# DeepRec-AI/HybridBackend

Hardware: AMD Instinct MI355X
Metric: M-lookups/sec, 26-col Criteo-shape dim16, 1/2/4/8 GPUs; % HBM roofline (higher is better)
Workload: dtype f32

## Files before the change

### hybridbackend_amd/_lib.py

```python
import ctypes as C
import os

_HERE = os.path.dirname(os.path.abspath(__file__))
LIB_PATH = os.environ.get('HBK_LIBRARY') or os.path.join(_HERE, 'lib', 'libhbk_core.so')

INT8, UINT8, INT32, UINT32, INT64, UINT64, HALF, FLOAT, DOUBLE = range(9)
APPLY_SGD, APPLY_ADAGRAD = 0, 2
APPLY_LAZY_ADAM, APPLY_FTRL, APPLY_ROWWISE_ADAGRAD = 3, 4, 5
GRAD_DETERMINISTIC = 1
COMBINER_SUM, COMBINER_MEAN, COMBINER_SQRTN = 0, 1, 2
OK, INVALID_ARGUMENT, UNIMPLEMENTED, INTERNAL = 0, 3, 12, 13
COMM_ID_BYTES = 128


class HbkError(RuntimeError):

  def __init__(self, code, message):
    super().__init__(f'[hbk status {code}] {message}')
    self.code = code


class InvalidArgumentError(HbkError, ValueError):
  pass

# ... 214 lines not shown


class StitchGradColumn(C.Structure):
  _fields_ = [('dim', C.c_int32), ('combiner', C.c_int32), ('n_ids', C.c_int64),
              ('index', C.c_void_p), ('row_splits', C.c_void_p), ('n_segments', C.c_int64),
              ('grad_out', C.c_void_p), ('grad_rows', C.c_void_p),
              ('run_start', C.c_void_p), ('run_base', C.c_void_p), ('n_runs', C.c_int32),
              ('grad_stride', C.c_int32), ('id_weights', C.c_void_p)]


_lib = None


def _declare(l):
  vp, i32, i64, sz = C.c_void_p, C.c_int32, C.c_int64, C.c_size_t
  protos = {
    'hbk_last_error': (C.c_char_p, []),
    'hbk_version': (C.c_char_p, []),
    'hbk_tables_layout': (C.c_size_t, [i32, vp, vp]),
    'hbk_tables_alloc': (C.c_int, [i32, vp, vp, vp]),
    'hbk_tables_free': (C.c_int, [vp]),
    'hbk_set_option': (C.c_int, [C.c_char_p, i32]),
    'hbk_get_option': (C.c_int, [C.c_char_p, vp]),
    'hbk_comm_rccl_ranks': (C.c_int, [vp]),
    'hbk_broadcast': (C.c_int, [vp, i32, vp, vp, i64, i32, vp]),
    'hbk_sharded_p2p_bind': (C.c_int, [vp, vp, vp, vp, vp]),
    'hbk_sharded_p2p_unbind': (C.c_int, [vp]),
    'hbk_sync_check': (C.c_int, []),
    'hbk_sync_check_stream': (C.c_int, [C.c_void_p]),
    'hbk_host_floormod_i64': (i64, [i64, i64]),
    'hbk_host_fastdiv_u64': (C.c_uint64, [C.c_uint64, C.c_uint64]),
    'hbk_host_crc32c': (C.c_uint32, [C.c_uint32, C.c_void_p, C.c_int64]),
    'hbk_host_xcd_contiguous': (i32, [i32, i32]),
    'hbk_floormod_n': (C.c_int, [i32, i32, vp, vp, vp, vp, vp]),
    'hbk_partition_workspace_bytes': (sz, [i32, vp, i32]),
    'hbk_partition_by_modulo_n': (C.c_int, [i32, i32, i32, vp, vp, vp, vp, vp, vp, sz, vp]),
    'hbk_partition_by_dual_modulo_n':
      (C.c_int, [i32, i32, i32, i32, i32, vp, vp, vp, vp, vp, vp, sz, vp]),
    'hbk_partition_by_modulo_host': (C.c_int, [i32, i32, i32, vp, vp, vp, vp, vp]),
    'hbk_partition_by_dual_modulo_host': (C.c_int, [i32, i32, i32, i32, i32, vp, vp, vp, vp, vp]),
    'hbk_cast_n': (C.c_int, [i32, i32, i32, vp, vp, vp, vp]),
    'hbk_unique_workspace_bytes': (sz, [i32, vp]),
    'hbk_unique_n': (C.c_int, [i32, vp, vp, vp, vp, vp, vp, sz, vp]),
    'hbk_group_lookup_fwd': (C.c_int, [i32, vp, vp]),
    'hbk_group_lookup_bwd_workspace_bytes': (sz, [i32, vp]),
    'hbk_group_lookup_bwd': (C.c_int, [i32, vp, C.c_float, vp, sz, vp]),
    'hbk_group_lookup_bwd_apply': (C.c_int, [i32, vp, i32, C.c_float, vp, sz, vp]),
    'hbk_group_lookup_bwd_adam_workspace_bytes': (sz, [i32, vp]),
    'hbk_group_lookup_bwd_adam': (C.c_int, [i32, vp, vp, vp, vp, C.c_float, vp, sz, vp]),
    'hbk_group_lookup_bwd_ftrl_workspace_bytes': (sz, [i32, vp]),
    'hbk_group_lookup_bwd_ftrl': (C.c_int, [i32, vp, vp, vp, vp, C.c_float, vp, sz, vp]),
    'hbk_group_lookup_fwd_clipped': (C.c_int, [i32, vp, vp, vp]),
    'hbk_group_lookup_bwd_apply_clipped_workspace_bytes': (sz, [i32, vp, vp]),
    'hbk_group_lookup_bwd_apply_clipped': (C.c_int, [i32, vp, vp, i32, C.c_float, vp, sz, vp]),
    'hbk_group_lookup_bwd_adam_clipped_workspace_bytes': (sz, [i32, vp, vp]),
    'hbk_group_lookup_bwd_adam_clipped': (C.c_int, [i32, vp, vp, vp, vp, vp, C.c_float, vp, sz, vp]),
    'hbk_group_lookup_bwd_ftrl_clipped_workspace_bytes': (sz, [i32, vp, vp]),
    'hbk_group_lookup_bwd_ftrl_clipped': (C.c_int, [i32, vp, vp, vp, vp, vp, C.c_float, vp, sz, vp]),
    'hbk_group_lookup_bwd_rowwise_adagrad_workspace_bytes': (sz, [i32, vp]),
    'hbk_group_lookup_bwd_rowwise_adagrad': (C.c_int, [i32, vp, vp, vp, C.c_float, vp, sz, vp]),
    'hbk_group_lookup_bwd_rowwise_adagrad_clipped_workspace_bytes': (sz, [i32, vp, vp]),
    'hbk_group_lookup_bwd_rowwise_adagrad_clipped': (C.c_int, [i32, vp, vp, vp, vp, C.c_float, vp, sz, vp]),
    'hbk_sparse_apply_slices_n': (C.c_int, [i32, vp, i32, vp, vp, vp, C.c_float, vp]),
    'hbk_lowp_lookup_fwd': (C.c_int, [i32, vp, vp]),
    'hbk_lowp_apply_slices_n': (C.c_int, [i32, vp, i32, vp, vp, vp, C.c_float, vp, vp]),
    'hbk_lowp_gather_rows_n': (C.c_int, [i32, vp, vp]),
# ... 254 lines not shown
```

### hybridbackend_amd/csrc/common.h

```cpp
#ifndef HBK_CSRC_COMMON_H_
#define HBK_CSRC_COMMON_H_

#include <hip/hip_runtime.h>
#include <stdarg.h>
#include <stdint.h>
#include <stdio.h>

#include "hbk.h"

namespace hbk {

int fail(int code, const char* fmt, ...);

#define HBK_HIP_OK(expr)                                                         \
  do {                                                                           \
    hipError_t e__ = (expr);                                                     \
    if (e__ != hipSuccess) {                                                     \
      return ::hbk::fail(HBK_INTERNAL, "%s failed: %s (%s:%d)", #expr,           \
                         hipGetErrorString(e__), __FILE__, __LINE__);            \
    }                                                                            \
  } while (0)

#define HBK_REQUIRE(cond, ...)                                                   \
  do {                                                                           \
// ... 51 lines not shown
  f.magic = m2 + 1;
  f.shift = k;
  f.kind = 2;
  return f;
}

__host__ __device__ inline uint64_t mulhi64(uint64_t a, uint64_t b) {
#if defined(__HIP_DEVICE_COMPILE__)
  return __umul64hi(a, b);
#else
  return (uint64_t)(((unsigned __int128)a * b) >> 64);
#endif
}

__host__ __device__ inline uint64_t fastdiv(uint64_t n, const FastDiv& f) {
  if (f.kind == 0) return n;
  if (f.kind == 1) return n >> f.shift;
  uint64_t t = mulhi64(f.magic, n);
  return (((n - t) >> 1) + t) >> f.shift;
}

__host__ __device__ inline uint64_t fastmod(uint64_t n, const FastDiv& f) {
  if (f.kind == 0) return 0;
  if (f.kind == 1) return n & (f.d - 1);
  return n - fastdiv(n, f) * f.d;
}

__host__ __device__ inline int xcd_contiguous(int b, int n, int on) {
  if (!on) return b;
  const int q = n >> 3, r = n & 7, x = b & 7, i = b >> 3;
  return (x < r ? x * (q + 1) : r * (q + 1) + (x - r) * q) + i;
}


__host__ __device__ inline uint64_t floormod_i64(int64_t v, const FastDiv& f) {
  uint64_t u = v < 0 ? (uint64_t)(~v) : (uint64_t)v;
  uint64_t r = fastmod(u, f);
  return v < 0 ? f.d - 1 - r : r;
}

struct Options {
  int bwd_buckets_log2 = -1;
  int bwd_bucket_pairs = 0;
  int bwd_split_pairs = 0;
  int bwd_onepass = 1;
  int fwd_xcd = 1;
  int bwd_xcd = 1;
  int bwd_wide = 1;
  int bwd_group_cols = 0;
  int bwd_dense = 1;
  int bwd_scatter_staged = 1;
  int bwd_rowsort_pos = 64;
  int bwd_pairs_packed = 1;
  int bwd_seg_inline = 1;
  int bwd_scale_fused = 1;
  int bwd_deterministic = 0;
  int bwd_simple = 1;
  int bwd_streams = 4;
  int bwd_lds_pad = 0;
  int bwd_trace = 0;
  int bwd_large_first = 0;
  int bwd_rowsort_ratio = 8;
  int bwd_weights_lds = 1;
  int fwd_d16 = 1;
  int fwd_interleave = 2;
  int fwd_hot_rows = 0;
  int unique_buckets_log2 = -1;
  int partition_sub_tiles = 1;
  int partition_fixed_max = 8;
  int partition_onepass = 1;
  int unique_onepass = 1;
  int sharded_groups = 0;
  int sharded_id64 = 0;
  int sharded_copy_self = 0;
  int sharded_trace = 0;
  int sharded_pack_early = 1;
  int sharded_wire_fused = 1;
  int sharded_inline = 1;
  int sharded_p2p = 1;
  int sharded_p2p_test_refuse = -1;
  int sync_wait_ms = 2000;
  int sync_onepass_off = 0;
  int sync_test_withhold = -1;
};
Options& options();

struct SyncTake {
  int32_t* words;
  int32_t* zero;
  int64_t zero_words;
  int32_t* status;
// ... 107 lines not shown
```

### hybridbackend_amd/csrc/lookup_bwd.hip

```cpp
#include <alloca.h>
#include <stdlib.h>
#include <string.h>

#include <algorithm>
#include <map>
#include <type_traits>
#include <mutex>
#include <vector>

#include "lookup_common.h"

namespace hbk {
size_t det_sort_temp_bytes(size_t n, int end_bit);
int det_sort_pairs(void* temp, size_t temp_bytes, const uint64_t* keys_in, uint64_t* keys_out,
                   const uint32_t* vals_in, uint32_t* vals_out, size_t n, int end_bit,
                   hipStream_t stream);
size_t det_scan_temp_bytes(size_t n);
int det_scan(void* temp, size_t temp_bytes, const int32_t* in, int32_t* out, size_t n,
             hipStream_t stream);
namespace {

constexpr int kBlock = 256;
constexpr int kWavesPerBlock = kBlock / kWave;
constexpr int kMaxCols = 64;
// ... 155 lines not shown
    rc.grad_delta = c.run_grads[rc.k] - start * c.dim;
  }
}

template <typename V>
__device__ inline void scale_segments(const GCol& c, const float* grad, int32_t stride, int combiner,
                                      int64_t s0, int n, const int32_t* sp) {
  constexpr int VE = sizeof(V) / 4;
  constexpr int kU = 4;
  const int tid = (int)threadIdx.x;
  const int sub = tid & ((1 << c.lpr_log2) - 1);
  const int groups = kBlock >> c.lpr_log2;
  if (sub >= c.chunks) return;
  for (int s = tid >> c.lpr_log2; s < n; s += kU * groups) {
    V g[kU];
    int32_t len[kU];
#pragma unroll
    for (int u = 0; u < kU; ++u) {
      const int ss = s + u * groups < n ? s + u * groups : n - 1;
      len[u] = s + u * groups < n ? sp[ss + 1] - sp[ss] : 0;
      g[u] = __builtin_nontemporal_load(reinterpret_cast<const V*>(
          grad + (s0 + ss) * (int64_t)stride + (int64_t)sub * VE));
    }
#pragma unroll
    for (int u = 0; u < kU; ++u) {
      if (len[u] <= 0) continue;
      const V v = combiner == HBK_COMBINER_MEAN ? g[u] / (float)len[u]
                                                : g[u] / sqrtf((float)len[u]);
      *reinterpret_cast<V*>(c.scaled + (s0 + s + u * groups) * (int64_t)c.dim + (int64_t)sub * VE) = v;
    }
  }
}

__device__ inline int32_t seg_search_wave(const int32_t* splits, int64_t n_seg, int32_t j) {
  const int lane = (int)threadIdx.x & (kWave - 1);
  int64_t lo = 0, n = n_seg;
  while (n > 1) {
    const int64_t step = (n + kWave - 1) / kWave;
    const int64_t s = lo + (int64_t)lane * step;
    const bool le = s < lo + n && splits[s] <= j;
    int k = (int)__builtin_popcountll(__ballot(le));
    if (k < 1) k = 1;
    const int64_t nlo = lo + (int64_t)(k - 1) * step;
    const int64_t rest = lo + n - nlo;
    lo = nlo;
    n = rest < step ? rest : step;
  }
  return (int32_t)lo;
}

__device__ inline int32_t tile_segments(const GCol& c, int64_t j_first, int64_t j_last,
                                        int32_t* seg_lds, int32_t* ends) {
  static_assert(kTile == kBlock * kPerThread && kPerThread % 4 == 0, "whole int4 per thread");
  const int tid = (int)threadIdx.x, lane = tid & (kWave - 1), wave = tid >> 6;
  if (wave == 0) {
    const int32_t s = seg_search_wave(c.splits, c.n_seg, (int32_t)j_first);
    if (tid == 0) ends[0] = s;
  } else if (wave == 1) {
    const int32_t s = seg_search_wave(c.splits, c.n_seg, (int32_t)j_last);
    if (tid == kWave) ends[1] = s;
  }
  int4* const v4 = reinterpret_cast<int4*>(seg_lds) + tid * (kPerThread / 4);
#pragma unroll
  for (int q = 0; q < kPerThread / 4; ++q) v4[q] = make_int4(0, 0, 0, 0);
  __syncthreads();
  const int32_t s_lo = ends[0], s_hi = ends[1];
  for (int32_t s = s_lo + 1 + tid; s <= s_hi; s += kBlock) {
    const int64_t p = (int64_t)c.splits[s] - j_first;
    if (p >= 0 && p < kTile) atomicAdd(&seg_lds[p], 1);
  }
  __syncthreads();
  int32_t x[kPerThread];
#pragma unroll
  for (int q = 0; q < kPerThread / 4; ++q) {
    const int4 v = v4[q];
    x[4 * q] = v.x;
    x[4 * q + 1] = v.y;
    x[4 * q + 2] = v.z;
    x[4 * q + 3] = v.w;
  }
#pragma unroll
  for (int q = 1; q < kPerThread; ++q) x[q] += x[q - 1];
  int32_t incl = x[kPerThread - 1];
#pragma unroll
  for (int o = 1; o < kWave; o <<= 1) {
    const int32_t y = __shfl_up(incl, o, kWave);
    if (lane >= o) incl += y;
  }
  if (lane == kWave - 1) ends[2 + wave] = incl;
  __syncthreads();
  int32_t before = incl - x[kPerThread - 1];
  for (int w = 0; w < wave; ++w) before += ends[2 + w];
#pragma unroll
  for (int q = 0; q < kPerThread / 4; ++q) {
    v4[q] = make_int4(x[4 * q] + before, x[4 * q + 1] + before, x[4 * q + 2] + before,
                      x[4 * q + 3] + before);
  }
  __syncthreads();
  return s_lo;
}

__global__ __launch_bounds__(kBlock) void bwd_segof_kernel(const GArgs a) {
  __shared__ int32_t sp[kBlock + 1];
  HBK_FIND_COL(a, segtile0)
  const int64_t s0 = ((int64_t)blockIdx.x - c.segtile0) * kBlock;
  const int tid = (int)threadIdx.x;
  const int n = c.n_seg - s0 < kBlock ? (int)(c.n_seg - s0) : kBlock;
  if (tid < n) sp[tid] = c.splits[s0 + tid];
  if (tid == 0) sp[n] = c.splits[s0 + n];
  __syncthreads();
  const int32_t lo = sp[0], hi = c.seg_of != nullptr ? sp[n] : sp[0];
  for (int32_t j = lo + tid; j < hi; j += kBlock) {
    int s = 0, e = n;
    while (e - s > 1) {
      const int mid = (s + e) >> 1;
      if (sp[mid] <= j) {
        s = mid;
      } else {
        e = mid;
      }
    }
    c.seg_of[j] = (int32_t)(s0 + s);
  }
  if (c.scaled != nullptr) {
    if (c.vec4) {
      scale_segments<f32x4>(c, c.grad_out, c.grad_stride, c.combiner, s0, n, sp);
    } else {
      scale_segments<float>(c, c.grad_out, c.grad_stride, c.combiner, s0, n, sp);
    }
  }
}
// ... 201 lines not shown
          seg[k] = c.seg_of[j];
        } else if (seg_inline) {
          seg[k] = s_lo + sp_lds[(k0 + k) * kBlock + tid];
        }
      }
    }
  };
  load_batch(0);
  for (int p = tid; p < P; p += kBlock) run[p] = c.bstart[p] + c.hist[(int64_t)ctile * P + p];
  __syncthreads();
  for (int k0 = 0; k0 < kPerThread; k0 += kBatch) {
    if (k0 > 0) load_batch(k0);
#pragma unroll
    for (int k = 0; k < kBatch; ++k) {
      const int64_t j = base + (int64_t)(k0 + k) * kBlock + tid;
      if (j < c.n_ids) {
        const uint64_t r = id_to_row(c.map, id[k]);
        if (r != kNoRow) {
          const int32_t pos = atomicAdd(&run[bucket_of(c, r)], 1);
          if (c.packed) {
            c.pair_row[0][pos] = (int64_t)((r << 32) | (uint64_t)(uint32_t)seg[k]);
          } else {
            c.pair_row[0][pos] = (int64_t)r;
            c.pair_seg[0][pos] = seg[k];
          }
        }
      }
    }
  }
}

constexpr int kStageMaxBuckets = 1024;

template <bool SIMPLE>
__global__ __launch_bounds__(kBlock, 4) void bwd_scatter_staged_kernel(const GArgs a) {
  extern __shared__ int32_t stage_dyn[];
  int32_t* const counters = stage_dyn;
  int32_t* const first = stage_dyn + a.stage_p;
  int32_t* const st_seg = stage_dyn + 2 * a.stage_p;
  __shared__ int64_t st_row[kTile];
  __shared__ uint16_t st_b[SIMPLE ? 1 : kTile];
  __shared__ int32_t wave_cnt[kWavesPerBlock];
  __shared__ int32_t n_staged;
  const int blk = xcd_contiguous((int)blockIdx.x, (int)gridDim.x, (a.xcd >> kXcdScatterBit) & 1);
  int ci;
  {
    const int l__ = (int)threadIdx.x & (kWave - 1);
    const int v__ = l__ < a.n_cols ? a.tile0[l__] : 0x7fffffff;
    ci = (int)__builtin_popcountll(__ballot(v__ <= blk)) - 1;
    ci = __builtin_amdgcn_readfirstlane(ci);
  }
  const GCol& c = a.col[ci];
  const int P = c.n_buckets;
  const int tid = (int)threadIdx.x, lane = tid & (kWave - 1), wave = tid >> 6;
  const int ctile = blk - c.tile0;
  const int64_t base = (int64_t)ctile * kTile;
  __shared__ int32_t seg_ends[2 + kWavesPerBlock];
  int32_t* const sp_lds = reinterpret_cast<int32_t*>(st_row);
  const bool seg_inline = c.splits != nullptr && (SIMPLE || c.seg_of == nullptr);
  RunCursor rc;
  int64_t id[kPerThread];
  int32_t seg[kPerThread];
#pragma unroll
  for (int k = 0; k < kPerThread; ++k) {
    const int64_t j = base + (int64_t)k * kBlock + tid;
    id[k] = 0;
    seg[k] = (int32_t)j;
    if (j < c.n_ids) {
      if (!SIMPLE && c.n_runs > 0) {
        run_seek(c, j, rc);
        if (!c.det) seg[k] = (int32_t)(uint32_t)(rc.grad_delta + j * c.dim);
      }
      id[k] = load_id(c.ids, SIMPLE ? 1 : c.ids64, SIMPLE ? j : j + rc.id_delta);
      if (!SIMPLE && c.seg_of != nullptr) seg[k] = c.seg_of[j];
    }
  }
  const int per = (P + kBlock - 1) / kBlock;
  const int beg = tid * per;
  const int end = beg + per < P ? beg + per : P;
  int32_t gpos[kStageMaxBuckets / kBlock];
#pragma unroll
  for (int q = 0; q < kStageMaxBuckets / kBlock; ++q) {
    const int p = beg + q;
    gpos[q] = q < per && p < end ? c.bstart[p] + c.hist[(int64_t)ctile * P + p] : 0;
  }
  if (seg_inline) {
    const int64_t j_last = (base + kTile < c.n_ids ? base + kTile : c.n_ids) - 1;
    const int32_t s_lo = tile_segments(c, base, j_last, sp_lds, seg_ends);
#pragma unroll
    for (int k = 0; k < kPerThread; ++k) seg[k] = s_lo + sp_lds[k * kBlock + tid];
  }
  for (int p = tid; p < P; p += kBlock) counters[p] = 0;
  __syncthreads();
  int32_t br[kPerThread];
#pragma unroll
  for (int k = 0; k < kPerThread; ++k) {
    const int64_t j = base + (int64_t)k * kBlock + tid;
    br[k] = -1;
    if (j < c.n_ids) {
      const uint64_t r = id_to_row(c.map, id[k]);
      id[k] = (int64_t)r;
      if (r != kNoRow) {
        const int b = SIMPLE ? (int)__umulhi((uint32_t)r, c.dense_mul) : bucket_of(c, r);
        br[k] = b | (atomicAdd(&counters[b], 1) << 10);
      }
    }
  }
  __syncthreads();
  int32_t sum_c = 0;
#pragma unroll
  for (int q = 0; q < kStageMaxBuckets / kBlock; ++q) {
    if (q < per && beg + q < end) sum_c += counters[beg + q];
  }
  int32_t incl_c = sum_c;
#pragma unroll
  for (int off = 1; off < kWave; off <<= 1) {
    const int32_t w = __shfl_up(incl_c, off, kWave);
    if (lane >= off) incl_c += w;
  }
  if (lane == kWave - 1) wave_cnt[wave] = incl_c;
  __syncthreads();
  int32_t run_c = incl_c - sum_c;
  for (int w = 0; w < wave; ++w) run_c += wave_cnt[w];
#pragma unroll
  for (int q = 0; q < kStageMaxBuckets / kBlock; ++q) {
    const int p = beg + q;
    if (q < per && p < end) {
      const int32_t n_c = counters[p];
      first[p] = run_c;
      counters[p] = gpos[q] - run_c;
      run_c += n_c;
    }
  }
  if (tid == kBlock - 1) n_staged = run_c;
  __syncthreads();
#pragma unroll
  for (int k = 0; k < kPerThread; ++k) {
    if (br[k] >= 0) {
      const int b = br[k] & 1023;
      const int L = first[b] + (br[k] >> 10);
      if (SIMPLE || c.packed) {
        st_row[L] = (int64_t)(((uint64_t)id[k] << 32) | (uint64_t)(uint32_t)seg[k]);
      } else {
        st_row[L] = id[k];
        st_seg[L] = seg[k];
      }
      if (!SIMPLE) st_b[L] = (uint16_t)b;
    }
  }
  __syncthreads();
  const int n_st = n_staged;
#pragma unroll
  for (int k = 0; k < kPerThread; ++k) {
    const int L = k * kBlock + tid;
    if (L < n_st) {
      const int sb = SIMPLE ? (int)__umulhi((uint32_t)((uint64_t)st_row[L] >> 32), c.dense_mul) : (int)st_b[L];
      const int32_t pos = counters[sb] + L;
      c.pair_row[0][pos] = st_row[L];
      if (!SIMPLE && !c.packed) c.pair_seg[0][pos] = st_seg[L];
    }
  }
}

#ifdef HBK_BWD_STAMPS
__device__ unsigned long long g_grp_trace[kTraceBlocks * kTraceSlots];
#define HBK_GSTAMP(i)                                                                       \
  do {                                                                                      \
    if (threadIdx.x == 0 && blockIdx.x < kTraceBlocks) {                                    \
      g_grp_trace[blockIdx.x * kTraceSlots + (i)] = __builtin_amdgcn_s_memrealtime();       \
    }                                                                                       \
  } while (0)
#else
#define HBK_GSTAMP(i)
#endif

constexpr int kGroupMaxBuckets = 2 * kBlock;

struct GSync {
  int32_t* hist;
  int32_t* zero;
  int64_t zero_words;
  SyncWait wait;
};

template <bool SIMPLE>
__global__ __launch_bounds__(kBlock, 4) void bwd_group_kernel(const GArgs a, const GSync y) {
  __shared__ int32_t counters[kGroupMaxBuckets];
  __shared__ int32_t tot_s[kGroupMaxBuckets], pre_s[kGroupMaxBuckets];
  __shared__ int64_t st_row[kTile];
  extern __shared__ int32_t st_seg[];
  __shared__ uint16_t st_b[kTile];
  __shared__ int32_t wave_tot[kWavesPerBlock], wave_cnt[kWavesPerBlock];
  __shared__ int32_t n_extra, gave_up, n_staged;
  const int tid = (int)threadIdx.x, lane = tid & (kWave - 1), wave = tid >> 6;
// ... 2358 lines not shown
    const unsigned tiles_p = (unsigned)((total + kDetTile - 1) / kDetTile);
    hipLaunchKernelGGL(det_heads_kernel, dim3(tiles_p), dim3(kBlock), 0, stream, a);
    HBK_HIP_OK(hipGetLastError());
    rc = det_scan(ws + l.temp, l.temp_bytes, heads, ranks, (size_t)total, stream);
    if (rc != HBK_OK) return rc;
    if (vec4) {
      det_launch_reduce<f32x4>(a, max_dim / 4, stream);
    } else {
      det_launch_reduce<float>(a, max_dim, stream);
    }
    HBK_HIP_OK(hipGetLastError());
    hipLaunchKernelGGL(det_counts_kernel, dim3(1), dim3(kWave), 0, stream, a);
    HBK_HIP_OK(hipGetLastError());
  }
  return HBK_OK;
}

}
}

#ifdef HBK_BWD_STAMPS
extern "C" int hbk_debug_grp_trace(unsigned long long* out, int reset) {
  using namespace hbk;
  HBK_HIP_OK(hipDeviceSynchronize());
  if (out != nullptr) {
    HBK_HIP_OK(hipMemcpyFromSymbol(out, HIP_SYMBOL(g_grp_trace), sizeof(g_grp_trace)));
  }
  if (reset) {
    static unsigned long long z[kTraceBlocks * kTraceSlots];
    HBK_HIP_OK(hipMemcpyToSymbol(HIP_SYMBOL(g_grp_trace), z, sizeof(z)));
  }
  return HBK_OK;
}
extern "C" int hbk_debug_bwd_sub(unsigned long long* out) {
  using namespace hbk;
  HBK_HIP_OK(hipDeviceSynchronize());
  HBK_HIP_OK(hipMemcpyFromSymbol(out, HIP_SYMBOL(g_bwd_sub), sizeof(g_bwd_sub)));
  return HBK_OK;
}
extern "C" int hbk_debug_bwd_trace(unsigned long long* out, int reset) {
  using namespace hbk;
  HBK_HIP_OK(hipDeviceSynchronize());
  if (out != nullptr) {
    HBK_HIP_OK(hipMemcpyFromSymbol(out, HIP_SYMBOL(g_bwd_trace), sizeof(g_bwd_trace)));
  }
  if (reset) {
    static unsigned long long z[kTraceBlocks * kTraceSlots];
    HBK_HIP_OK(hipMemcpyToSymbol(HIP_SYMBOL(g_bwd_trace), z, sizeof(z)));
  }
  return HBK_OK;
}
#endif

extern "C" size_t hbk_group_lookup_bwd_workspace_bytes(int32_t n_cols,
                                                       const hbk_lookup_grad_column_t* cols) {
  if (n_cols <= 0 || cols == nullptr) return 0;
  if (hbk::any_weighted(n_cols, cols)) {
    std::vector<hbk_lookup_grad_column_t> as_sum;
    const size_t tb = hbk::weighted_as_sum(n_cols, cols, nullptr, &as_sum);
    return tb + hbk_group_lookup_bwd_workspace_bytes(n_cols, as_sum.data());
  }
  std::vector<hbk::ColInfo> info;
  for (int32_t c = 0; c < n_cols; ++c) info.push_back(hbk::col_info(cols[c]));
  return hbk::call_layout(n_cols, cols, info).total;
}

// ... 383 lines not shown
                   c.dense_mul != 0;
    unpacked = unpacked || c.packed == 0;
  }
  const size_t lds_tail = (unpacked ? (size_t)kTile * 4 : 0) + (size_t)options().bwd_lds_pad * 1024;
  memset(sync, 0, sizeof(*sync));
  const auto group_kernel = simple_group ? &bwd_group_kernel<true> : &bwd_group_kernel<false>;
  bool onepass = g.onepass && g.sync_words < (1ll << 30);
  if (onepass) {
    SyncTake take;
    onepass = sync_take(ls, (size_t)g.sync_words, &take, reinterpret_cast<const void*>(group_kernel), kBlock,
                        64, caller);
    if (onepass) {
      sync->hist = take.words;
      sync->zero = take.zero;
      sync->zero_words = take.zero_words;
      sync->wait = sync_wait_of(take);
    }
  }
  if (onepass) {
    SyncChain chain(ls);
    hipLaunchKernelGGL(group_kernel, tiles, block, lds_tail, ls, args, *sync);
    return true;
  }
  hipLaunchKernelGGL(simple_group ? &bwd_hist_kernel<true> : &bwd_hist_kernel<false>, tiles, block, g.lds_hist,
                     ls, args);
  if (g.small_scan) {
    hipLaunchKernelGGL(bwd_scan_fused_kernel, dim3((unsigned)k), block, 0, ls, args);
  } else {
    hipLaunchKernelGGL(bwd_scan_tiles_kernel, dim3((unsigned)g.scans), block, 0, ls, args);
    hipLaunchKernelGGL(bwd_scan_kernel, dim3((unsigned)k), block, 0, ls, args);
  }
  if (g.lds_hist <= (size_t)4 * kStageMaxBuckets && options().bwd_scatter_staged != 0) {
    args.stage_p = (int32_t)(g.lds_hist / 4);
    hipLaunchKernelGGL(simple_group ? &bwd_scatter_staged_kernel<true> : &bwd_scatter_staged_kernel<false>,
                       tiles, block, 2 * g.lds_hist + lds_tail, ls, args);
  } else {
    hipLaunchKernelGGL(bwd_scatter_pairs_kernel, tiles, block, g.lds_hist, ls, args);
  }
  return false;
}

int launch_reduce_merge(const Group& g, bool det, int32_t apply, float apply_lr, const int4* desc,
                        const int32_t* poison, hipStream_t ls) {
  const GArgs& args = g.args;
  const int step = apply_lr == 0.0f ? 0 : apply == HBK_APPLY_ADAGRAD ? 2 : 1;
  typedef void (*reduce_fn)(const GArgs, const int4*, int, int, const int32_t*);
  typedef void (*merge_fn)(const GArgs, int, const int32_t*);
#define HBK_BY_STEP(K, V, ...) {&K<V, 0, ##__VA_ARGS__>, &K<V, 1, ##__VA_ARGS__>, &K<V, 2, ##__VA_ARGS__>}
  static const reduce_fn kReduce[kKinds][3] = {
      HBK_BY_STEP(bwd_dense_kernel, f32x4, false), HBK_BY_STEP(bwd_dense_kernel, float, false),
      HBK_BY_STEP(bwd_dense_kernel, f32x4, true), HBK_BY_STEP(bwd_dense_kernel, float, true),
      HBK_BY_STEP(bwd_reduce_kernel, f32x4, false), HBK_BY_STEP(bwd_reduce_kernel, float, false),
      {nullptr, &bwd_reduce_kernel<f32x4, 1, true>, &bwd_reduce_kernel<f32x4, 2, true>},
      {nullptr, &bwd_reduce_kernel<float, 1, true>, &bwd_reduce_kernel<float, 2, true>},
      HBK_BY_STEP(bwd_rowsort_kernel, f32x4), HBK_BY_STEP(bwd_rowsort_kernel, float)};
  static const merge_fn kMerge[kKinds][3] = {
      HBK_BY_STEP(bwd_dense_merge_kernel, f32x4), HBK_BY_STEP(bwd_dense_merge_kernel, float),
      HBK_BY_STEP(bwd_dense_merge_kernel, f32x4), HBK_BY_STEP(bwd_dense_merge_kernel, float),
      HBK_BY_STEP(bwd_merge_kernel, f32x4, false), HBK_BY_STEP(bwd_merge_kernel, float, false),
      {nullptr, &bwd_merge_kernel<f32x4, 1, true>, &bwd_merge_kernel<f32x4, 2, true>},
      {nullptr, &bwd_merge_kernel<float, 1, true>, &bwd_merge_kernel<float, 2, true>},
      HBK_BY_STEP(bwd_rowsort_merge_kernel, f32x4), HBK_BY_STEP(bwd_rowsort_merge_kernel, float)};
  static const reduce_fn kReduceDet[2][3] = {HBK_BY_STEP(bwd_rowsort_kernel, f32x4, true),
                                             HBK_BY_STEP(bwd_rowsort_kernel, float, true)};
#undef HBK_BY_STEP
  int status = HBK_OK;
  if (det) {
    hipLaunchKernelGGL(bwd_rowsort_count_kernel, dim3((unsigned)g.buckets), dim3(kBlock), 0, ls, args, desc,
// ... 229 lines not shown
```

### hybridbackend_amd/csrc/misc.cpp

```cpp
#include <stdlib.h>
#include <string.h>

#include <vector>

#include "common.h"

namespace hbk {
namespace {
thread_local char g_last_error[1024] = "";
}

int fail(int code, const char* fmt, ...) {
  va_list ap;
  va_start(ap, fmt);
  vsnprintf(g_last_error, sizeof(g_last_error), fmt, ap);
  va_end(ap);
  return code;
}
}

namespace hbk {
namespace {
struct OptionEntry {
  const char* name;
  const char* env;
  int Options::*field;
};
const OptionEntry kOptions[] = {
    {"bwd_buckets_log2", "HBK_BWD_LOG2P", &Options::bwd_buckets_log2},
    {"bwd_bucket_pairs", "HBK_BWD_TARGET", &Options::bwd_bucket_pairs},
    {"bwd_split_pairs", "HBK_BWD_SPLIT", &Options::bwd_split_pairs},
    {"bwd_onepass", "HBK_BWD_ONEPASS", &Options::bwd_onepass},
    {"bwd_group_cols", "HBK_BWD_GROUP_COLS", &Options::bwd_group_cols},
    {"bwd_dense", "HBK_BWD_DENSE", &Options::bwd_dense},
    {"bwd_scatter_staged", "HBK_BWD_SCATTER_STAGED", &Options::bwd_scatter_staged},
    {"bwd_rowsort_pos", "HBK_BWD_ROWSORT_POS", &Options::bwd_rowsort_pos},
    {"bwd_rowsort_ratio", "HBK_BWD_ROWSORT_RATIO", &Options::bwd_rowsort_ratio},
    {"bwd_deterministic", "HBK_BWD_DETERMINISTIC", &Options::bwd_deterministic},
    {"bwd_streams", "HBK_BWD_STREAMS", &Options::bwd_streams},
    {"bwd_trace", "HBK_BWD_TRACE", &Options::bwd_trace},
    {"bwd_lds_pad", "HBK_BWD_LDS_PAD", &Options::bwd_lds_pad},
    {"bwd_large_first", "HBK_BWD_LARGE_FIRST", &Options::bwd_large_first},
    {"bwd_pairs_packed", "HBK_BWD_PAIRS_PACKED", &Options::bwd_pairs_packed},
    {"bwd_seg_inline", "HBK_BWD_SEG_INLINE", &Options::bwd_seg_inline},
    {"bwd_scale_fused", "HBK_BWD_SCALE_FUSED", &Options::bwd_scale_fused},
    {"bwd_simple", "HBK_BWD_SIMPLE", &Options::bwd_simple},
    {"fwd_d16", "HBK_FWD_D16", &Options::fwd_d16},
    {"bwd_weights_lds", "HBK_BWD_WEIGHTS_LDS", &Options::bwd_weights_lds},
    {"bwd_wide", "HBK_BWD_WIDE", &Options::bwd_wide},
    {"bwd_xcd", "HBK_BWD_XCD", &Options::bwd_xcd},
    {"fwd_xcd", "HBK_FWD_XCD", &Options::fwd_xcd},
    {"fwd_hot_rows", "HBK_FWD_HOT", &Options::fwd_hot_rows},
    {"fwd_interleave", "HBK_FWD_INTERLEAVE", &Options::fwd_interleave},
    {"unique_buckets_log2", "HBK_UNIQUE_LOG2P", &Options::unique_buckets_log2},
    {"partition_sub_tiles", "HBK_PART_SUB", &Options::partition_sub_tiles},
    {"partition_fixed_max", "HBK_PART_FIXED", &Options::partition_fixed_max},
    {"partition_onepass", "HBK_PART_ONEPASS", &Options::partition_onepass},
    {"unique_onepass", "HBK_UNIQUE_ONEPASS", &Options::unique_onepass},
    {"sharded_groups", "HBK_SHARDED_GROUPS", &Options::sharded_groups},
    {"sharded_id64", "HBK_SHARDED_ID64", &Options::sharded_id64},
    {"sharded_copy_self", "HBK_SHARDED_COPY_SELF", &Options::sharded_copy_self},
    {"sharded_trace", "HBK_SHARDED_TRACE", &Options::sharded_trace},
    {"sharded_inline", "HBK_SHARDED_INLINE", &Options::sharded_inline},
    {"sharded_p2p", "HBK_SHARDED_P2P", &Options::sharded_p2p},
    {"sharded_p2p_test_refuse", "HBK_SHARDED_P2P_TEST_REFUSE", &Options::sharded_p2p_test_refuse},
    {"sharded_wire_fused", "HBK_SHARDED_WIRE_FUSED", &Options::sharded_wire_fused},
    {"sharded_pack_early", "HBK_SHARDED_PACK_EARLY", &Options::sharded_pack_early},
    {"sync_wait_ms", "HBK_SYNC_WAIT_MS", &Options::sync_wait_ms},
// ... 71 lines not shown
  if (n == 0) return HBK_OK;
  std::vector<size_t> off((size_t)n);
  const size_t total = hbk_tables_layout(n, bytes, off.data());
  void* p = nullptr;
  const hipError_t e = hipMalloc(&p, total > 0 ? total : 1);
  if (e != hipSuccess) {
    (void)hipGetLastError();
    return fail(HBK_INTERNAL, "tables_alloc: hipMalloc of %zu bytes failed: %s", total,
                hipGetErrorString(e));
  }
  for (int32_t i = 0; i < n; ++i) tables[i] = static_cast<char*>(p) + off[(size_t)i];
  *slab = p;
  return HBK_OK;
}
extern "C" int hbk_tables_free(void* slab) {
  using namespace hbk;
  if (slab == nullptr) return HBK_OK;
  const hipError_t e = hipFree(slab);
  if (e != hipSuccess) return fail(HBK_INTERNAL, "tables_free: %s", hipGetErrorString(e));
  return HBK_OK;
}

extern "C" int64_t hbk_host_floormod_i64(int64_t v, int64_t d) {
  if (d <= 0) return -1;
  hbk::FastDiv f = hbk::make_fastdiv((uint64_t)d);
  f.d = (uint64_t)d;
  return (int64_t)hbk::floormod_i64(v, f);
}

extern "C" int32_t hbk_host_xcd_contiguous(int32_t block, int32_t n_blocks) {
  return hbk::xcd_contiguous(block, n_blocks, 1);
}

extern "C" uint64_t hbk_host_fastdiv_u64(uint64_t n, uint64_t d) {
  if (d == 0) return 0;
  hbk::FastDiv f = hbk::make_fastdiv(d);
  return hbk::fastdiv(n, f);
}

extern "C" uint32_t hbk_host_crc32c(uint32_t crc, const void* data, int64_t n) {
  struct Tables {
    uint32_t t[8][256];
    Tables() {
      for (uint32_t i = 0; i < 256; ++i) {
        uint32_t c = i;
        for (int k = 0; k < 8; ++k) c = (c & 1u) ? (c >> 1) ^ 0x82f63b78u : c >> 1;
        t[0][i] = c;
      }
      for (uint32_t i = 0; i < 256; ++i) {
        for (int s = 1; s < 8; ++s) t[s][i] = (t[s - 1][i] >> 8) ^ t[0][t[s - 1][i] & 0xffu];
      }
    }
  };
  static const Tables tab;
  const uint8_t* p = static_cast<const uint8_t*>(data);
  uint32_t l = ~crc;
  if (p == nullptr || n <= 0) return crc;
  while (n > 0 && (reinterpret_cast<uintptr_t>(p) & 7u) != 0) {
    l = tab.t[0][(l ^ *p++) & 0xffu] ^ (l >> 8);
    --n;
  }
  while (n >= 8) {
    uint64_t w;
    memcpy(&w, p, 8);
    const uint32_t lo = (uint32_t)w ^ l, hi = (uint32_t)(w >> 32);
    l = tab.t[7][lo & 0xffu] ^ tab.t[6][(lo >> 8) & 0xffu] ^ tab.t[5][(lo >> 16) & 0xffu] ^
// ... 12 lines not shown
```

### include/hbk.h

```cpp
#ifndef HBK_H_
#define HBK_H_

#include <stddef.h>
#include <stdint.h>

#ifdef __cplusplus
extern "C" {
#endif

typedef void* hbk_stream_t;

#define HBK_OK 0
#define HBK_INVALID_ARGUMENT 3
#define HBK_UNIMPLEMENTED 12
#define HBK_INTERNAL 13

#define HBK_INT8 0
#define HBK_UINT8 1
#define HBK_INT32 2
#define HBK_UINT32 3
#define HBK_INT64 4
#define HBK_UINT64 5
#define HBK_HALF 6
#define HBK_FLOAT 7
#define HBK_DOUBLE 8

#define HBK_COMBINER_SUM 0
#define HBK_COMBINER_MEAN 1
#define HBK_COMBINER_SQRTN 2

#define HBK_TOPOLOGY_ALL 0
#define HBK_TOPOLOGY_INTRA_NODE 1
#define HBK_TOPOLOGY_INTER_NODE 2

const char* hbk_last_error(void);
const char* hbk_version(void);

size_t hbk_tables_layout(int32_t n, const size_t* bytes, size_t* offsets);
int hbk_tables_alloc(int32_t n, const size_t* bytes, void** tables, void** slab);
int hbk_tables_free(void* slab);
int hbk_set_option(const char* name, int32_t value);
int hbk_get_option(const char* name, int32_t* value);
int hbk_sync_check(void);
int hbk_sync_check_stream(hbk_stream_t stream);
int64_t hbk_host_floormod_i64(int64_t v, int64_t d);
uint64_t hbk_host_fastdiv_u64(uint64_t n, uint64_t d);
int32_t hbk_host_xcd_contiguous(int32_t block, int32_t n_blocks);
uint32_t hbk_host_crc32c(uint32_t crc, const void* data, int64_t n);

int hbk_floormod_n(int32_t n_cols, int32_t dtype, const void* const* inputs,
                   const int64_t* lens, const int64_t* buckets, void* const* outputs,
                   hbk_stream_t stream);

size_t hbk_partition_workspace_bytes(int32_t n_cols, const int64_t* lens,
                                     int32_t num_partitions);
int hbk_partition_by_modulo_n(int32_t n_cols, int32_t dtype, int32_t num_partitions,
                              const void* const* inputs, const int64_t* lens,
                              void* const* outputs, int32_t* const* sizes,
                              int32_t* const* indices, void* workspace,
                              size_t workspace_bytes, hbk_stream_t stream);

int hbk_partition_by_dual_modulo_n(int32_t n_cols, int32_t dtype, int32_t num_partitions,
                                   int32_t modulus, int32_t stage,
                                   const void* const* inputs, const int64_t* lens,
                                   void* const* outputs, int32_t* const* sizes,
                                   int32_t* const* indices, void* workspace,
                                   size_t workspace_bytes, hbk_stream_t stream);
int hbk_partition_by_modulo_host(int32_t n_cols, int32_t dtype, int32_t num_partitions,
                                 const void* const* inputs, const int64_t* lens,
                                 void* const* outputs, int32_t* const* sizes,
                                 int32_t* const* indices);
int hbk_partition_by_dual_modulo_host(int32_t n_cols, int32_t dtype, int32_t num_partitions,
                                      int32_t modulus, int32_t stage,
                                      const void* const* inputs, const int64_t* lens,
                                      void* const* outputs, int32_t* const* sizes,
                                      int32_t* const* indices);

int hbk_cast_n(int32_t n, int32_t src_dtype, int32_t dst_dtype, const void* const* inputs,
               const int64_t* lens, void* const* outputs, hbk_stream_t stream);

// ... 694 lines not shown
```

Measured before the change: 30630.

## Make staged backward scatter kernel persistent with next-tile prefetch

Converts the staged backward scatter kernel from one block per tile into a persistent grid sized to the resident block count. Each block walks several tiles using an XCD-aware walk, strided by default. In the simple path it issues the next tile's id loads and segment search while the current tile is being written out, to hide load latency. It also raises the launch-bounds occupancy hint and swaps the shuffle-based scan for ds_bpermute. This adds register pressure, loop and synchronisation overhead, and gives up some parallelism when there are few tiles.

```diff
diff --git a/hybridbackend_amd/_lib.py b/hybridbackend_amd/_lib.py
--- a/hybridbackend_amd/_lib.py
+++ b/hybridbackend_amd/_lib.py
@@ -270,6 +270,7 @@
     'hbk_host_fastdiv_u64': (C.c_uint64, [C.c_uint64, C.c_uint64]),
     'hbk_host_crc32c': (C.c_uint32, [C.c_uint32, C.c_void_p, C.c_int64]),
     'hbk_host_xcd_contiguous': (i32, [i32, i32]),
+    'hbk_host_persistent_walk': (None, [i32, i32, i32, i32, i32, vp]),
     'hbk_floormod_n': (C.c_int, [i32, i32, vp, vp, vp, vp, vp]),
     'hbk_partition_workspace_bytes': (sz, [i32, vp, i32]),
     'hbk_partition_by_modulo_n': (C.c_int, [i32, i32, i32, vp, vp, vp, vp, vp, vp, sz, vp]),
diff --git a/hybridbackend_amd/csrc/common.h b/hybridbackend_amd/csrc/common.h
--- a/hybridbackend_amd/csrc/common.h
+++ b/hybridbackend_amd/csrc/common.h
@@ -107,6 +107,32 @@
   return (x < r ? x * (q + 1) : r * (q + 1) + (x - r) * q) + i;
 }
 
+struct ItemWalk {
+  int first, step, count;
+};
+__host__ __device__ inline ItemWalk persistent_walk(int b, int grid, int n, int on, int contiguous) {
+  int xs = 0, len = n, w = grid, i = b;
+  if (on && grid >= 8) {
+    const int q = n >> 3, r = n & 7, x = b & 7;
+    i = b >> 3;
+    xs = x < r ? x * (q + 1) : r * (q + 1) + (x - r) * q;
+    len = q + (x < r ? 1 : 0);
+    w = (grid >> 3) + (x < (grid & 7) ? 1 : 0);
+  }
+  ItemWalk k;
+  if (contiguous) {
+    const int lo = (int)((long long)i * len / w), hi = (int)((long long)(i + 1) * len / w);
+    k.first = xs + lo;
+    k.step = 1;
+    k.count = hi - lo;
+  } else {
+    k.first = xs + i;
+    k.step = w;
+    k.count = i < len ? (len - i + w - 1) / w : 0;
+  }
+  return k;
+}
+
 
 __host__ __device__ inline uint64_t floormod_i64(int64_t v, const FastDiv& f) {
   uint64_t u = v < 0 ? (uint64_t)(~v) : (uint64_t)v;
@@ -132,6 +158,7 @@
   int bwd_deterministic = 0;
   int bwd_simple = 1;
   int bwd_streams = 4;
+  int bwd_scatter_walk = 0;
   int bwd_lds_pad = 0;
   int bwd_trace = 0;
   int bwd_large_first = 0;
diff --git a/hybridbackend_amd/csrc/lookup_bwd.hip b/hybridbackend_amd/csrc/lookup_bwd.hip
--- a/hybridbackend_amd/csrc/lookup_bwd.hip
+++ b/hybridbackend_amd/csrc/lookup_bwd.hip
@@ -211,8 +211,8 @@
   }
 }
 
-__device__ inline int32_t seg_search_wave(const int32_t* splits, int64_t n_seg, int32_t j) {
-  const int lane = (int)threadIdx.x & (kWave - 1);
+__device__ inline int32_t seg_search_wave(const int32_t* splits, int64_t n_seg, int32_t j,
+                                          int lane = (int)threadIdx.x & (kWave - 1)) {
   int64_t lo = 0, n = n_seg;
   while (n > 1) {
     const int64_t step = (n + kWave - 1) / kWave;
@@ -228,22 +228,38 @@
   return (int32_t)lo;
 }
 
-__device__ inline int32_t tile_segments(const GCol& c, int64_t j_first, int64_t j_last,
-                                        int32_t* seg_lds, int32_t* ends) {
-  static_assert(kTile == kBlock * kPerThread && kPerThread % 4 == 0, "whole int4 per thread");
-  const int tid = (int)threadIdx.x, lane = tid & (kWave - 1), wave = tid >> 6;
+__device__ inline void tile_segment_ends(const GCol& c, int64_t j_first, int64_t j_last, int32_t* ends,
+                                         int tid = (int)threadIdx.x) {
+  const int wave = tid >> 6, lane = tid & (kWave - 1);
   if (wave == 0) {
-    const int32_t s = seg_search_wave(c.splits, c.n_seg, (int32_t)j_first);
+    const int32_t s = seg_search_wave(c.splits, c.n_seg, (int32_t)j_first, lane);
     if (tid == 0) ends[0] = s;
   } else if (wave == 1) {
-    const int32_t s = seg_search_wave(c.splits, c.n_seg, (int32_t)j_last);
+    const int32_t s = seg_search_wave(c.splits, c.n_seg, (int32_t)j_last, lane);
     if (tid == kWave) ends[1] = s;
   }
+}
+
+__device__ inline void tile_segments_clear(int32_t* seg_lds, int tid = (int)threadIdx.x) {
+  static_assert(kTile == kBlock * kPerThread && kPerThread % 4 == 0, "whole int4 per thread");
   int4* const v4 = reinterpret_cast<int4*>(seg_lds) + tid * (kPerThread / 4);
 #pragma unroll
   for (int q = 0; q < kPerThread / 4; ++q) v4[q] = make_int4(0, 0, 0, 0);
-  __syncthreads();
-  const int32_t s_lo = ends[0], s_hi = ends[1];
+}
+
+__device__ inline int32_t wave_inclusive_sum(int32_t v, int lane) {
+#pragma unroll
+  for (int o = 1; o < kWave; o <<= 1) {
+    const int32_t y = __builtin_amdgcn_ds_bpermute((lane >= o ? lane - o : lane) << 2, v);
+    if (lane >= o) v += y;
+  }
+  return v;
+}
+
+__device__ inline void tile_segment_counts(const GCol& c, int64_t j_first, int32_t s_lo, int32_t s_hi,
+                                           int32_t* seg_lds, int32_t* wave_tot, int tid = (int)threadIdx.x) {
+  const int lane = tid & (kWave - 1), wave = tid >> 6;
+  int4* const v4 = reinterpret_cast<int4*>(seg_lds) + tid * (kPerThread / 4);
   for (int32_t s = s_lo + 1 + tid; s <= s_hi; s += kBlock) {
     const int64_t p = (int64_t)c.splits[s] - j_first;
     if (p >= 0 && p < kTile) atomicAdd(&seg_lds[p], 1);
@@ -260,22 +276,26 @@
   }
 #pragma unroll
   for (int q = 1; q < kPerThread; ++q) x[q] += x[q - 1];
-  int32_t incl = x[kPerThread - 1];
-#pragma unroll
-  for (int o = 1; o < kWave; o <<= 1) {
-    const int32_t y = __shfl_up(incl, o, kWave);
-    if (lane >= o) incl += y;
-  }
-  if (lane == kWave - 1) ends[2 + wave] = incl;
+  const int32_t incl = wave_inclusive_sum(x[kPerThread - 1], lane);
+  if (lane == kWave - 1) wave_tot[wave] = incl;
   __syncthreads();
   int32_t before = incl - x[kPerThread - 1];
-  for (int w = 0; w < wave; ++w) before += ends[2 + w];
+  for (int w = 0; w < wave; ++w) before += wave_tot[w];
 #pragma unroll
   for (int q = 0; q < kPerThread / 4; ++q) {
     v4[q] = make_int4(x[4 * q] + before, x[4 * q + 1] + before, x[4 * q + 2] + before,
                       x[4 * q + 3] + before);
   }
   __syncthreads();
+}
+
+__device__ inline int32_t tile_segments(const GCol& c, int64_t j_first, int64_t j_last,
+                                        int32_t* seg_lds, int32_t* ends) {
+  tile_segment_ends(c, j_first, j_last, ends);
+  tile_segments_clear(seg_lds);
+  __syncthreads();
+  const int32_t s_lo = ends[0], s_hi = ends[1];
+  tile_segment_counts(c, j_first, s_lo, s_hi, seg_lds, ends + 2);
   return s_lo;
 }
 
@@ -543,8 +563,32 @@
 
 constexpr int kStageMaxBuckets = 1024;
 
+#ifdef HBK_BWD_STAMPS
+__device__ unsigned long long g_sct_trace[kTraceBlocks * kTraceSlots];
+#define HBK_SSTAMP_BEGIN()                                                     \
+  unsigned long long st_acc__[kTraceSlots] = {0, 0, 0, 0, 0, 0, 0, 0};         \
+  unsigned long long st_prev__ = __builtin_amdgcn_s_memrealtime();
+#define HBK_SSTAMP(i)                                                          \
+  do {                                                                         \
+    const unsigned long long n__ = __builtin_amdgcn_s_memrealtime();           \
+    st_acc__[i] += n__ - st_prev__;                                            \
+    st_prev__ = n__;                                                           \
+  } while (0)
+#define HBK_SSTAMP_END()                                                       \
+  if (threadIdx.x == 0 && blockIdx.x < kTraceBlocks) {                         \
+    for (int i__ = 0; i__ < kTraceSlots; ++i__) {                              \
+      g_sct_trace[blockIdx.x * kTraceSlots + i__] = st_acc__[i__];             \
+    }                                                                          \
+  }
+#else
+#define HBK_SSTAMP_BEGIN()
+#define HBK_SSTAMP(i)
+#define HBK_SSTAMP_END()
+#endif
+
 template <bool SIMPLE>
-__global__ __launch_bounds__(kBlock, 4) void bwd_scatter_staged_kernel(const GArgs a) {
+__global__ __launch_bounds__(kBlock, SIMPLE ? 8 : 7) void bwd_scatter_staged_kernel(const GArgs a, const int n_tiles,
+                                                                      const int contiguous) {
   extern __shared__ int32_t stage_dyn[];
   int32_t* const counters = stage_dyn;
   int32_t* const first = stage_dyn + a.stage_p;
@@ -553,124 +597,181 @@
   __shared__ uint16_t st_b[SIMPLE ? 1 : kTile];
   __shared__ int32_t wave_cnt[kWavesPerBlock];
   __shared__ int32_t n_staged;
-  const int blk = xcd_contiguous((int)blockIdx.x, (int)gridDim.x, (a.xcd >> kXcdScatterBit) & 1);
+  __shared__ int32_t seg_ends[2];
+  __shared__ int32_t seg_tot[kWavesPerBlock];
+  int32_t* const sp_lds = reinterpret_cast<int32_t*>(st_row);
+  const ItemWalk walk = persistent_walk((int)blockIdx.x, (int)gridDim.x, n_tiles,
+                                        (a.xcd >> kXcdScatterBit) & 1, contiguous);
+  if (walk.count <= 0) return;
+  auto col_after = [&](int ci_, int t) {
+    while (ci_ + 1 < a.n_cols && a.tile0[ci_ + 1] <= t) ++ci_;
+    return ci_;
+  };
+  int64_t idn[kPerThread];
+  int32_t segn[SIMPLE ? 1 : kPerThread];
+  auto issue = [&](const GCol& cn, int ctile, int tid) {
+    const int64_t base = (int64_t)ctile * kTile;
+    RunCursor rc;
+#pragma unroll
+    for (int k = 0; k < kPerThread; ++k) {
+      const int64_t j = base + (int64_t)k * kBlock + tid;
+      idn[k] = 0;
+      if (!SIMPLE) segn[k] = (int32_t)j;
+      if (j < cn.n_ids) {
+        if (!SIMPLE && cn.n_runs > 0) {
+          run_seek(cn, j, rc);
+          if (!cn.det) segn[k] = (int32_t)(uint32_t)(rc.grad_delta + j * cn.dim);
+        }
+        idn[k] = load_id(cn.ids, SIMPLE ? 1 : cn.ids64, SIMPLE ? j : j + rc.id_delta);
+        if (!SIMPLE && cn.seg_of != nullptr) segn[k] = cn.seg_of[j];
+      }
+    }
+  };
+  auto search = [&](const GCol& cn, int ctile, int tid) {
+    if (cn.splits != nullptr && (SIMPLE || cn.seg_of == nullptr)) {
+      const int64_t base = (int64_t)ctile * kTile;
+      tile_segment_ends(cn, base, (base + kTile < cn.n_ids ? base + kTile : cn.n_ids) - 1, seg_ends, tid);
+    }
+  };
+  HBK_SSTAMP_BEGIN()
+  int tile = walk.first, left = walk.count;
   int ci;
   {
     const int l__ = (int)threadIdx.x & (kWave - 1);
     const int v__ = l__ < a.n_cols ? a.tile0[l__] : 0x7fffffff;
-    ci = (int)__builtin_popcountll(__ballot(v__ <= blk)) - 1;
+    ci = (int)__builtin_popcountll(__ballot(v__ <= tile)) - 1;
     ci = __builtin_amdgcn_readfirstlane(ci);
   }
-  const GCol& c = a.col[ci];
-  const int P = c.n_buckets;
-  const int tid = (int)threadIdx.x, lane = tid & (kWave - 1), wave = tid >> 6;
-  const int ctile = blk - c.tile0;
-  const int64_t base = (int64_t)ctile * kTile;
-  __shared__ int32_t seg_ends[2 + kWavesPerBlock];
-  int32_t* const sp_lds = reinterpret_cast<int32_t*>(st_row);
-  const bool seg_inline = c.splits != nullptr && (SIMPLE || c.seg_of == nullptr);
-  RunCursor rc;
-  int64_t id[kPerThread];
-  int32_t seg[kPerThread];
-#pragma unroll
-  for (int k = 0; k < kPerThread; ++k) {
-    const int64_t j = base + (int64_t)k * kBlock + tid;
-    id[k] = 0;
-    seg[k] = (int32_t)j;
-    if (j < c.n_ids) {
-      if (!SIMPLE && c.n_runs > 0) {
-        run_seek(c, j, rc);
-        if (!c.det) seg[k] = (int32_t)(uint32_t)(rc.grad_delta + j * c.dim);
-      }
-      id[k] = load_id(c.ids, SIMPLE ? 1 : c.ids64, SIMPLE ? j : j + rc.id_delta);
-      if (!SIMPLE && c.seg_of != nullptr) seg[k] = c.seg_of[j];
-    }
-  }
-  const int per = (P + kBlock - 1) / kBlock;
-  const int beg = tid * per;
-  const int end = beg + per < P ? beg + per : P;
-  int32_t gpos[kStageMaxBuckets / kBlock];
-#pragma unroll
-  for (int q = 0; q < kStageMaxBuckets / kBlock; ++q) {
-    const int p = beg + q;
-    gpos[q] = q < per && p < end ? c.bstart[p] + c.hist[(int64_t)ctile * P + p] : 0;
-  }
-  if (seg_inline) {
-    const int64_t j_last = (base + kTile < c.n_ids ? base + kTile : c.n_ids) - 1;
-    const int32_t s_lo = tile_segments(c, base, j_last, sp_lds, seg_ends);
-#pragma unroll
-    for (int k = 0; k < kPerThread; ++k) seg[k] = s_lo + sp_lds[k * kBlock + tid];
-  }
-  for (int p = tid; p < P; p += kBlock) counters[p] = 0;
-  __syncthreads();
-  int32_t br[kPerThread];
-#pragma unroll
-  for (int k = 0; k < kPerThread; ++k) {
-    const int64_t j = base + (int64_t)k * kBlock + tid;
-    br[k] = -1;
-    if (j < c.n_ids) {
-      const uint64_t r = id_to_row(c.map, id[k]);
-      id[k] = (int64_t)r;
-      if (r != kNoRow) {
-        const int b = SIMPLE ? (int)__umulhi((uint32_t)r, c.dense_mul) : bucket_of(c, r);
-        br[k] = b | (atomicAdd(&counters[b], 1) << 10);
-      }
-    }
-  }
-  __syncthreads();
-  int32_t sum_c = 0;
-#pragma unroll
-  for (int q = 0; q < kStageMaxBuckets / kBlock; ++q) {
-    if (q < per && beg + q < end) sum_c += counters[beg + q];
-  }
-  int32_t incl_c = sum_c;
-#pragma unroll
-  for (int off = 1; off < kWave; off <<= 1) {
-    const int32_t w = __shfl_up(incl_c, off, kWave);
-    if (lane >= off) incl_c += w;
-  }
-  if (lane == kWave - 1) wave_cnt[wave] = incl_c;
-  __syncthreads();
-  int32_t run_c = incl_c - sum_c;
-  for (int w = 0; w < wave; ++w) run_c += wave_cnt[w];
-#pragma unroll
-  for (int q = 0; q < kStageMaxBuckets / kBlock; ++q) {
-    const int p = beg + q;
-    if (q < per && p < end) {
-      const int32_t n_c = counters[p];
-      first[p] = run_c;
-      counters[p] = gpos[q] - run_c;
-      run_c += n_c;
-    }
-  }
-  if (tid == kBlock - 1) n_staged = run_c;
-  __syncthreads();
-#pragma unroll
-  for (int k = 0; k < kPerThread; ++k) {
-    if (br[k] >= 0) {
-      const int b = br[k] & 1023;
-      const int L = first[b] + (br[k] >> 10);
-      if (SIMPLE || c.packed) {
-        st_row[L] = (int64_t)(((uint64_t)id[k] << 32) | (uint64_t)(uint32_t)seg[k]);
-      } else {
-        st_row[L] = id[k];
-        st_seg[L] = seg[k];
-      }
-      if (!SIMPLE) st_b[L] = (uint16_t)b;
-    }
-  }
-  __syncthreads();
-  const int n_st = n_staged;
-#pragma unroll
-  for (int k = 0; k < kPerThread; ++k) {
-    const int L = k * kBlock + tid;
-    if (L < n_st) {
-      const int sb = SIMPLE ? (int)__umulhi((uint32_t)((uint64_t)st_row[L] >> 32), c.dense_mul) : (int)st_b[L];
-      const int32_t pos = counters[sb] + L;
-      c.pair_row[0][pos] = st_row[L];
-      if (!SIMPLE && !c.packed) c.pair_seg[0][pos] = st_seg[L];
-    }
-  }
+  constexpr bool kAhead = SIMPLE;
+  if (kAhead) {
+    issue(a.col[ci], tile - a.col[ci].tile0, (int)threadIdx.x);
+    search(a.col[ci], tile - a.col[ci].tile0, (int)threadIdx.x);
+    __syncthreads();
+  }
+  HBK_SSTAMP(7);
+  for (;;) {
+    int tid = (int)threadIdx.x;
+    asm volatile("" : "+v"(tid));
+    tid &= kBlock - 1;
+    const int lane = tid & (kWave - 1), wave = tid >> 6;
+    const GCol& c = a.col[ci];
+    const int P = c.n_buckets;
+    const int ctile = tile - c.tile0;
+    const int64_t base = (int64_t)ctile * kTile;
+    const bool seg_inline = c.splits != nullptr && (SIMPLE || c.seg_of == nullptr);
+    if (!kAhead) {
+      issue(c, ctile, tid);
+      search(c, ctile, tid);
+      __syncthreads();
+    }
+    const int32_t s_lo = seg_inline ? seg_ends[0] : 0, s_hi = seg_inline ? seg_ends[1] : 0;
+    const int per = (P + kBlock - 1) / kBlock;
+    const int beg = tid * per;
+    const int end = beg + per < P ? beg + per : P;
+    int32_t gb[kStageMaxBuckets / kBlock], gh[kStageMaxBuckets / kBlock];
+#pragma unroll
+    for (int q = 0; q < kStageMaxBuckets / kBlock; ++q) {
+      const int p = beg + q;
+      const bool mine = q < per && p < end;
+      gb[q] = mine ? c.bstart[p] : 0;
+      gh[q] = mine ? c.hist[(int64_t)ctile * P + p] : 0;
+    }
+    --left;
+    int32_t seg[kPerThread];
+    for (int p = tid; p < P; p += kBlock) counters[p] = 0;
+    if (seg_inline) {
+      tile_segments_clear(sp_lds, tid);
+      __syncthreads();
+      tile_segment_counts(c, base, s_lo, s_hi, sp_lds, seg_tot, tid);
+#pragma unroll
+      for (int k = 0; k < kPerThread; ++k) seg[k] = s_lo + sp_lds[k * kBlock + tid];
+    } else {
+      __syncthreads();
+#pragma unroll
+      for (int k = 0; k < kPerThread; ++k) seg[k] = SIMPLE ? (int32_t)(base + (int64_t)k * kBlock + tid) : segn[k];
+    }
+    int32_t gpos[kStageMaxBuckets / kBlock];
+#pragma unroll
+    for (int q = 0; q < kStageMaxBuckets / kBlock; ++q) gpos[q] = gb[q] + gh[q];
+    HBK_SSTAMP(1);
+    int32_t br[kPerThread];
+#pragma unroll
+    for (int k = 0; k < kPerThread; ++k) {
+      const int64_t j = base + (int64_t)k * kBlock + tid;
+      br[k] = -1;
+      if (j < c.n_ids) {
+        const uint64_t r = id_to_row(c.map, idn[k]);
+        idn[k] = (int64_t)r;
+        if (r != kNoRow) {
+          const int b = SIMPLE ? (int)__umulhi((uint32_t)r, c.dense_mul) : bucket_of(c, r);
+          br[k] = b | (atomicAdd(&counters[b], 1) << 10);
+        }
+      }
+    }
+    __syncthreads();
+    HBK_SSTAMP(2);
+    int32_t sum_c = 0;
+#pragma unroll
+    for (int q = 0; q < kStageMaxBuckets / kBlock; ++q) {
+      if (q < per && beg + q < end) sum_c += counters[beg + q];
+    }
+    const int32_t incl_c = wave_inclusive_sum(sum_c, lane);
+    if (lane == kWave - 1) wave_cnt[wave] = incl_c;
+    __syncthreads();
+    int32_t run_c = incl_c - sum_c;
+    for (int w = 0; w < wave; ++w) run_c += wave_cnt[w];
+#pragma unroll
+    for (int q = 0; q < kStageMaxBuckets / kBlock; ++q) {
+      const int p = beg + q;
+      if (q < per && p < end) {
+        const int32_t n_c = counters[p];
+        first[p] = run_c;
+        counters[p] = gpos[q] - run_c;
+        run_c += n_c;
+      }
+    }
+    if (tid == kBlock - 1) n_staged = run_c;
+    __syncthreads();
+    HBK_SSTAMP(3);
+#pragma unroll
+    for (int k = 0; k < kPerThread; ++k) {
+      if (br[k] >= 0) {
+        const int b = br[k] & 1023;
+        const int L = first[b] + (br[k] >> 10);
+        if (SIMPLE || c.packed) {
+          st_row[L] = (int64_t)(((uint64_t)idn[k] << 32) | (uint64_t)(uint32_t)seg[k]);
+        } else {
+          st_row[L] = idn[k];
+          st_seg[L] = seg[k];
+        }
+        if (!SIMPLE) st_b[L] = (uint16_t)b;
+      }
+    }
+    __syncthreads();
+    HBK_SSTAMP(4);
+    if (left > 0) {
+      tile += walk.step;
+      ci = col_after(ci, tile);
+      if (kAhead) issue(a.col[ci], tile - a.col[ci].tile0, tid);
+    }
+    const int n_st = n_staged;
+#pragma unroll
+    for (int k = 0; k < kPerThread; ++k) {
+      const int L = k * kBlock + tid;
+      if (L < n_st) {
+        const int sb = SIMPLE ? (int)__umulhi((uint32_t)((uint64_t)st_row[L] >> 32), c.dense_mul) : (int)st_b[L];
+        const int32_t pos = counters[sb] + L;
+        c.pair_row[0][pos] = st_row[L];
+        if (!SIMPLE && !c.packed) c.pair_seg[0][pos] = st_seg[L];
+      }
+    }
+    HBK_SSTAMP(5);
+    if (left == 0) break;
+    if (kAhead) search(a.col[ci], tile - a.col[ci].tile0, tid);
+    __syncthreads();
+    HBK_SSTAMP(6);
+  }
+  HBK_SSTAMP_END()
 }
 
 #ifdef HBK_BWD_STAMPS
@@ -3095,6 +3196,18 @@
   }
   return HBK_OK;
 }
+extern "C" int hbk_debug_sct_trace(unsigned long long* out, int reset) {
+  using namespace hbk;
+  HBK_HIP_OK(hipDeviceSynchronize());
+  if (out != nullptr) {
+    HBK_HIP_OK(hipMemcpyFromSymbol(out, HIP_SYMBOL(g_sct_trace), sizeof(g_sct_trace)));
+  }
+  if (reset) {
+    static unsigned long long z[kTraceBlocks * kTraceSlots];
+    HBK_HIP_OK(hipMemcpyToSymbol(HIP_SYMBOL(g_sct_trace), z, sizeof(z)));
+  }
+  return HBK_OK;
+}
 extern "C" int hbk_debug_bwd_sub(unsigned long long* out) {
   using namespace hbk;
   HBK_HIP_OK(hipDeviceSynchronize());
@@ -3544,8 +3657,11 @@
   }
   if (g.lds_hist <= (size_t)4 * kStageMaxBuckets && options().bwd_scatter_staged != 0) {
     args.stage_p = (int32_t)(g.lds_hist / 4);
+    const int64_t resident = (int64_t)(simple_group ? 8 : 7) * device_cus();
+    const int64_t grid = g.tiles < resident ? (g.tiles > 0 ? g.tiles : 1) : resident;
     hipLaunchKernelGGL(simple_group ? &bwd_scatter_staged_kernel<true> : &bwd_scatter_staged_kernel<false>,
-                       tiles, block, 2 * g.lds_hist + lds_tail, ls, args);
+                       dim3((unsigned)grid), block, 2 * g.lds_hist + lds_tail, ls, args, (int)g.tiles,
+                       options().bwd_scatter_walk);
   } else {
     hipLaunchKernelGGL(bwd_scatter_pairs_kernel, tiles, block, g.lds_hist, ls, args);
   }
diff --git a/hybridbackend_amd/csrc/misc.cpp b/hybridbackend_amd/csrc/misc.cpp
--- a/hybridbackend_amd/csrc/misc.cpp
+++ b/hybridbackend_amd/csrc/misc.cpp
@@ -34,6 +34,7 @@
     {"bwd_group_cols", "HBK_BWD_GROUP_COLS", &Options::bwd_group_cols},
     {"bwd_dense", "HBK_BWD_DENSE", &Options::bwd_dense},
     {"bwd_scatter_staged", "HBK_BWD_SCATTER_STAGED", &Options::bwd_scatter_staged},
+    {"bwd_scatter_walk", "HBK_BWD_SCATTER_WALK", &Options::bwd_scatter_walk},
     {"bwd_rowsort_pos", "HBK_BWD_ROWSORT_POS", &Options::bwd_rowsort_pos},
     {"bwd_rowsort_ratio", "HBK_BWD_ROWSORT_RATIO", &Options::bwd_rowsort_ratio},
     {"bwd_deterministic", "HBK_BWD_DETERMINISTIC", &Options::bwd_deterministic},
@@ -171,6 +172,14 @@
   return hbk::xcd_contiguous(block, n_blocks, 1);
 }
 
+extern "C" void hbk_host_persistent_walk(int32_t block, int32_t grid, int32_t n, int32_t xcd, int32_t contiguous,
+                                         int32_t* out) {
+  const hbk::ItemWalk w = hbk::persistent_walk(block, grid, n, xcd, contiguous);
+  out[0] = w.first;
+  out[1] = w.step;
+  out[2] = w.count;
+}
+
 extern "C" uint64_t hbk_host_fastdiv_u64(uint64_t n, uint64_t d) {
   if (d == 0) return 0;
   hbk::FastDiv f = hbk::make_fastdiv(d);
diff --git a/include/hbk.h b/include/hbk.h
--- a/include/hbk.h
+++ b/include/hbk.h
@@ -46,6 +46,8 @@
 int64_t hbk_host_floormod_i64(int64_t v, int64_t d);
 uint64_t hbk_host_fastdiv_u64(uint64_t n, uint64_t d);
 int32_t hbk_host_xcd_contiguous(int32_t block, int32_t n_blocks);
+void hbk_host_persistent_walk(int32_t block, int32_t grid, int32_t n, int32_t xcd, int32_t contiguous,
+                              int32_t* out);
 uint32_t hbk_host_crc32c(uint32_t crc, const void* data, int64_t n);
 
 int hbk_floormod_n(int32_t n_cols, int32_t dtype, const void* const* inputs,
```

After: 30610. Within noise of the previous version (-0.1%).
